# Alxaline/BraTS21

Measured on AMD Instinct MI355X. Metric: train patches/sec (4x128^3, width-48), higher is better.
Workload: dtype bf16; 1 GPU; equiunet width=48, batch=2/GPU of 4x128^3 synthetic patches, fwd + deep-supervision Dice + bwd + ranger (BASELINE.json configs[1]); global_batch=2, parallelism=dp1

## Files before the change

brats21_amd/csrc/gen_twin_dispatch.py:

```python
#!/usr/bin/env python3
import re
import sys

BOTH = {"brats_conv3d_set_vs8", "brats_conv3d_set_kp", "brats_conv3d_set_wgrad_alltaps", "brats_conv3d_set_x3_wgrad_fused"}
DATA = {"brats_conv3d_f8_fwd", "brats_conv3d_wgrad_f8", "brats_conv3d_pack_weights_multi"}

txt = re.sub(r"/\*.*?\*/", " ", open(sys.argv[1]).read(), flags=re.S)
protos = {}
for m in re.finditer(r"(const char\s*\*|size_t|int)\s+(brats_[a-z0-9_]+)\s*\(([^)]*)\)\s*;", txt):
    protos[m.group(2)] = (" ".join(m.group(1).split()), " ".join(m.group(3).split()))
names = []
for path in sys.argv[2:]:
    for m in re.finditer(r'extern "C" [a-z_ \*]+?BRATS_API\((brats_[a-z0-9_]+)\)\(', open(path).read()):
        names.append(m.group(1))
print("// GENERATED by gen_twin_dispatch.py from include/brats_hip.h -- do not edit")
print('#include "../../include/brats_hip.h"')
print('extern "C" {')
for n in names:
    if n not in protos:
        raise SystemExit(f"{n} is defined in a twinned translation unit but not declared in brats_hip.h")
    ret, args = protos[n]
    arglist = [] if args in ("", "void") else [a.strip() for a in args.split(",")]
    argnames = [re.search(r"([A-Za-z_][A-Za-z0-9_]*)$", a).group(1) for a in arglist]
    call = ", ".join(argnames)
    sig = args if arglist else "void"
    print(f"{ret} {n}_bf16({sig});")
    print(f"{ret} {n}_f16({sig});")
    if n in DATA:
        if n + "_f16" not in protos:
            raise SystemExit(f"{n}_f16 must be declared in brats_hip.h (16-bit data, no dtype argument)")
        print(f"{ret} {n}({sig}) {{ return {n}_bf16({call}); }}")
    elif n in BOTH:
        print(f"{ret} {n}({sig}) {{ {n}_f16({call}); return {n}_bf16({call}); }}")
    elif "dtype" in argnames:
        call16 = ", ".join("BRATS_BF16" if a == "dtype" else a for a in argnames)
        callx3 = ", ".join("BRATS_X3_BF16" if a == "dtype" else a for a in argnames)
        print(f"{ret} {n}({sig}) {{ return dtype == BRATS_F16 ? {n}_f16({call16}) : dtype == BRATS_X3_F16 ? {n}_f16({callx3}) : {n}_bf16({call}); }}")
# ... 4 lines not shown
```

brats21_amd/csrc/head.hip:

```cpp
#include "twin_begin.hpp"
#include "common.hpp"

int brats_lerp_adjoint_f32_planes(const float* in, float* out, size_t outer, int Lout, int Lin, size_t inner, hipStream_t st);

static inline int sgrid(size_t total, int block) {
  size_t b = (total + block - 1) / block;
  return (int)(b < 1 ? 1 : (b > 8192 ? 8192 : b));
}
constexpr int HEAD_KMAX = 4;

struct HeadPre { const float* scale_shift; float nslope; int evo; };
DEVI float head_pre(float x, float sc, float sh, const HeadPre& pre) {
  if (pre.evo) return x * __builtin_amdgcn_rcpf(1.f + __expf(-x)) * sc + sh;
  const float p = x * sc + sh;
  return p > 0.f ? p : p * pre.nslope;
}
template <typename T, bool PRE = false>
__global__ void head_conv_kernel(const T* __restrict__ x, int xpitch, const float* __restrict__ w, const float* __restrict__ b,
                                 float* __restrict__ low, int C, int K, size_t voxels, HeadPre pre) {
  constexpr int VW = 16 / sizeof(T);
  extern __shared__ float sm[];
  float* ws = sm;
  float* red = sm + HEAD_KMAX * C;
  for (int i = threadIdx.x; i < K * C; i += blockDim.x) ws[i] = w[i];
  __syncthreads();
  const int n = blockIdx.y;
  const int cv = C / VW, vl_n = blockDim.x / cv;
  const int mycv = threadIdx.x % cv, myvl = threadIdx.x / cv, c0 = mycv * VW;
  const T* xb = x + (size_t)n * voxels * xpitch;
  float psc[VW], psh[VW];
  if constexpr (PRE) {
#pragma unroll
    for (int j = 0; j < VW; ++j) {
      const bool in = myvl < vl_n;
      psc[j] = in ? pre.scale_shift[((size_t)n * C + c0 + j) * 2] : 0.f;
      psh[j] = in ? pre.scale_shift[((size_t)n * C + c0 + j) * 2 + 1] : 0.f;
// ... 101 lines not shown
      for (int i = 0; i < 4; ++i) { xb0[i] = pre_act(xb0[i], 0); xb1[i] = pre_act(xb1[i], 1); }
    }
#pragma unroll
    for (int i = 0; i < 4; ++i) {
      f32x4 acc = {0.f, 0.f, 0.f, 0.f};
#pragma unroll
      for (int part = 2; part >= 0; --part) {
        acc = MFMA16_16x16x32(wa[part][0], xb0[i], acc);
        acc = MFMA16_16x16x32(wa[part][1], xb1[i], acc);
      }
      const size_t vv = v0 + 16 * i + v;
      if (q == 0 && vv < voxels) {
#pragma unroll
        for (int r = 0; r < 4; ++r)
          if (r < K) lowp[(size_t)r * voxels + vv] = acc[r] + bias[r];
      }
    }
  }
}

struct Lerp { int i0, i1; float w0, w1; };
DEVI Lerp lerp_coef(int o, int in_len, float scale) {
  const float src = scale * (float)o;
  Lerp l;
  l.i0 = (int)src;
  if (l.i0 > in_len - 1) l.i0 = in_len - 1;
  l.i1 = l.i0 + (l.i0 < in_len - 1 ? 1 : 0);
  l.w1 = fminf(fmaxf(src - (float)l.i0, 0.f), 1.f);
  l.w0 = 1.f - l.w1;
  return l;
}
static inline float ac_scale(int in_len, int out_len) { return out_len > 1 ? (float)(in_len - 1) / (float)(out_len - 1) : 0.f; }

__global__ void __launch_bounds__(256) upsample_planes_kernel(const float* __restrict__ low, float* __restrict__ out, int D, int H, int W, int sc,
                                                              float sd, float sh, float sw) {
  const int Ho = H * sc, Wo = W * sc, Do = D * sc, W4 = Wo / 4;
  const int zo = blockIdx.y;
  const size_t pl = blockIdx.z;
  const Lerp lz = lerp_coef(zo, D, sd);
  const float* p0 = low + pl * D * H * W + (size_t)lz.i0 * H * W;
  const float* p1 = low + pl * D * H * W + (size_t)lz.i1 * H * W;
  float* o = out + (pl * Do + zo) * (size_t)Ho * Wo;
  for (int it = blockIdx.x * blockDim.x + threadIdx.x; it < Ho * W4; it += gridDim.x * blockDim.x) {
    const int yo = it / W4, x0 = (it % W4) * 4;
    const Lerp ly = lerp_coef(yo, H, sh);
    f32x4 r;
#pragma unroll
    for (int j = 0; j < 4; ++j) {
      const Lerp lx = lerp_coef(x0 + j, W, sw);
      float acc = 0.f;
#pragma unroll
      for (int k = 0; k < 8; ++k) {
        const float* p = (k & 4) ? p1 : p0;
        const int yy = (k & 2) ? ly.i1 : ly.i0, xx = (k & 1) ? lx.i1 : lx.i0;
        const float wgt = ((k & 4) ? lz.w1 : lz.w0) * ((k & 2) ? ly.w1 : ly.w0) * ((k & 1) ? lx.w1 : lx.w0);
        acc += wgt * p[yy * W + xx];
      }
      r[j] = acc;
    }
    *(f32x4*)(o + (size_t)yo * Wo + x0) = r;
  }
}

template <bool PRE>
static int head_conv_launch(const void* x, int xpitch, const float* w, const float* b, float* low, int dtype, int N, int C, int K,
                            size_t vox, HeadPre pre, hipStream_t st) {
  const int vw = dtype == BRATS_BF16 ? 8 : 4;
  const int cvh = C / vw, vlh = 256 / cvh;
  if (cvh > 256) BRATS_FAIL(BRATS_E_UNSUPPORTED, "head_fwd: C too large");
  dim3 grid(sgrid((vox + vlh - 1) / vlh, 1), N);
  const size_t ldsh = (size_t)(HEAD_KMAX * C + 256 * HEAD_KMAX) * sizeof(float);
  if (dtype == BRATS_BF16 && C <= 64 && (double)vox * xpitch * 2 < 2147483648.0) {
    const size_t waves = (vox + 63) / 64;
    const unsigned gx = (unsigned)(waves / 4 < 1 ? 1 : (waves / 4 > 8192 ? 8192 : waves / 4));
    hipLaunchKernelGGL(head_conv_mfma_kernel<PRE>, dim3(gx, N), dim3(256), 0, st, (const bf16_t*)x, xpitch, w, b, low, C, K, vox, pre);
  } else if (dtype == BRATS_BF16)
    hipLaunchKernelGGL((head_conv_kernel<bf16_t, PRE>), grid, dim3(256), ldsh, st, (const bf16_t*)x, xpitch, w, b, low, C, K, vox, pre);
  else
    hipLaunchKernelGGL((head_conv_kernel<float, PRE>), grid, dim3(256), ldsh, st, (const float*)x, xpitch, w, b, low, C, K, vox, pre);
  BRATS_CHECK_LAUNCH();
  return 0;
}

extern "C" int BRATS_API(brats_gn_head_fwd)(const void* y, int ypitch, const float* scale_shift, int act, float slope, const float* w,
                                 const float* b, float* out, int dtype, int N, int C, int K, int voxels, brats_stream_t s) {
  const int vw = dtype == BRATS_BF16 ? 8 : 4;
  if (!y || !scale_shift || !w || !out || K < 1 || K > HEAD_KMAX || C % vw || ypitch % vw)
    BRATS_FAIL(BRATS_E_ARG, "gn_head_fwd: bad argument (K<=4, C multiple of %d)", vw);
  if (act > BRATS_ACT_LEAKY) BRATS_FAIL(BRATS_E_UNSUPPORTED, "gn_head_fwd: relu / leakyrelu only (act=%d)", act);
  return head_conv_launch<true>(y, ypitch, w, b, out, dtype, N, C, K, (size_t)voxels,
                                HeadPre{scale_shift, act == BRATS_ACT_RELU ? 0.f : slope, 0}, (hipStream_t)s);
}

extern "C" int BRATS_API(brats_evonorm_head_fwd)(const void* y, int ypitch, const float* scale_shift, const float* w, const float* b,
                                      float* out, int dtype, int N, int C, int K, int voxels, brats_stream_t s) {
  const int vw = dtype == BRATS_BF16 ? 8 : 4;
  if (!y || !scale_shift || !w || !out || K < 1 || K > HEAD_KMAX || C % vw || ypitch % vw)
    BRATS_FAIL(BRATS_E_ARG, "evonorm_head_fwd: bad argument (K<=4, C multiple of %d)", vw);
  return head_conv_launch<true>(y, ypitch, w, b, out, dtype, N, C, K, (size_t)voxels, HeadPre{scale_shift, 0.f, 1}, (hipStream_t)s);
}

extern "C" int BRATS_API(brats_head_fwd)(const void* x, int xpitch, const float* w, const float* b, float* lowres, float* out,
                              int dtype, int N, int C, int K, int D, int H, int W, int scale, brats_stream_t s) {
  const int vw = dtype == BRATS_BF16 ? 8 : 4;
  if (!x || !w || !out || K < 1 || K > HEAD_KMAX || C % vw || xpitch % vw || scale < 1)
    BRATS_FAIL(BRATS_E_ARG, "head_fwd: bad argument (K<=4, C multiple of %d)", vw);
  if (scale > 1 && !lowres) BRATS_FAIL(BRATS_E_ARG, "head_fwd: lowres workspace required when scale > 1");
  hipStream_t st = (hipStream_t)s;
  const size_t vox = (size_t)D * H * W;
  float* low = scale > 1 ? lowres : out;
  if (int rc = head_conv_launch<false>(x, xpitch, w, b, low, dtype, N, C, K, vox, HeadPre{nullptr, 0.f, 0}, st)) return rc;
  if (scale > 1) {
    if ((W * scale) % 4) BRATS_FAIL(BRATS_E_UNSUPPORTED, "head_fwd: up-sampled width %d must be a multiple of 4", W * scale);
    const int items = H * scale * (W * scale / 4);
    hipLaunchKernelGGL(upsample_planes_kernel, dim3((unsigned)((items + 255) / 256), (unsigned)(D * scale), (unsigned)(N * K)), dim3(256), 0, st,
                       (const float*)low, out, D, H, W, scale, ac_scale(D, D * scale), ac_scale(H, H * scale), ac_scale(W, W * scale));
  }
  BRATS_CHECK_LAUNCH();
  return 0;
}

template <typename T>
__global__ void __launch_bounds__(256) head_bwd_kernel(const T* __restrict__ x, int xpitch, const float* __restrict__ w, const float* __restrict__ dlow,
                                T* __restrict__ dx, int dxpitch, float* __restrict__ dw , int C, int K,
                                size_t voxels) {
  constexpr int VW = 16 / sizeof(T);
  extern __shared__ float sm[];
  float* ws = sm;
  for (int i = threadIdx.x; i < K * C; i += blockDim.x) ws[i] = w[i];
  __syncthreads();
  const int n = blockIdx.y;
  const int cv = C / VW, vl_n = blockDim.x / cv;
  const int mycv = threadIdx.x % cv, myvl = threadIdx.x / cv, c0 = mycv * VW;
  float aw[HEAD_KMAX][VW];
  float ab[HEAD_KMAX];
#pragma unroll
  for (int k = 0; k < HEAD_KMAX; ++k) {
    ab[k] = 0.f;
#pragma unroll
    for (int j = 0; j < VW; ++j) aw[k][j] = 0.f;
  }
  if (myvl < vl_n) {
    const T* xb = x + (size_t)n * voxels * xpitch + c0;
    T* dxb = dx ? dx + (size_t)n * voxels * dxpitch + c0 : nullptr;
    float wr[HEAD_KMAX][VW];
#pragma unroll
    for (int k = 0; k < HEAD_KMAX; ++k)
#pragma unroll
      for (int j = 0; j < VW; ++j) wr[k][j] = k < K ? ws[k * C + c0 + j] : 0.f;
// ... 57 lines not shown
  if ((int)threadIdx.x < K) {
    float t = 0.f;
    for (int l = 0; l < vl_n; ++l) t += scr[vl_n * K * C + l * K + threadIdx.x];
    part[K * C + threadIdx.x] = t;
  }
}

constexpr int HEAD_MAX_BLOCKS = 1024;
static size_t head_lerp_floats(int N, int K, int D, int H, int W, int scale) {
  if (scale <= 1) return 0;
  const size_t p = (size_t)N * K;
  const size_t dlow = p * D * H * W, t1 = p * D * (H * scale) * (W * scale), t2 = p * D * H * (W * scale);
  return dlow + t1 + t2;
}
extern "C" size_t BRATS_API(brats_head_bwd_ws_bytes)(int N, int C, int K, int D, int H, int W, int scale) {
  return (head_lerp_floats(N, K, D, H, W, scale) + (size_t)(N * HEAD_MAX_BLOCKS + 1) * (K * C + K)) * sizeof(float);
}

extern "C" int BRATS_API(brats_head_bwd)(const void* x, int xpitch, const float* w, const float* dout, float* ws, void* dx, int dxpitch,
                              float* dw, float* db, int dtype, int N, int C, int K, int D, int H, int W, int scale,
                              brats_stream_t s) {
  const int vw = dtype == BRATS_BF16 ? 8 : 4;
  if (!x || !w || !dout || !dw || !db || K < 1 || K > HEAD_KMAX || C % vw || xpitch % vw || (dx && dxpitch % vw) ||
      C / vw > 128)
    BRATS_FAIL(BRATS_E_ARG, "head_bwd: bad argument");
  if (!ws) BRATS_FAIL(BRATS_E_ARG, "head_bwd: workspace required");
  hipStream_t st = (hipStream_t)s;
  const size_t vox = (size_t)D * H * W, p = (size_t)N * K;
  const float* dlow = dout;
  if (scale > 1) {
    float* dl = ws;
    float* t1 = dl + p * vox;
    float* t2 = t1 + p * D * (H * scale) * (W * scale);
    int rc;
    if ((rc = brats_lerp_adjoint_f32_planes(dout, t1, p, D * scale, D, (size_t)H * scale * W * scale, st))) return rc;
    if ((rc = brats_lerp_adjoint_f32_planes(t1, t2, p * D, H * scale, H, (size_t)W * scale, st))) return rc;
    if ((rc = brats_lerp_adjoint_f32_planes(t2, dl, p * D * H, W * scale, W, 1, st))) return rc;
    dlow = dl;
  }
  const int cv = C / vw, vl = 256 / cv;
  size_t gx = (vox + (size_t)vl * 16 - 1) / ((size_t)vl * 16);
  dim3 grid((unsigned)(gx < 1 ? 1 : (gx > HEAD_MAX_BLOCKS ? HEAD_MAX_BLOCKS : gx)), N);
  const size_t lds = (size_t)(K * C + vl * K * C + vl * K) * sizeof(float);
  float* part = ws + head_lerp_floats(N, K, D, H, W, scale);
  float* tot = part + (size_t)N * HEAD_MAX_BLOCKS * (K * C + K);
  if (dtype == BRATS_BF16)
    hipLaunchKernelGGL(head_bwd_kernel<bf16_t>, grid, dim3(256), lds, st, (const bf16_t*)x, xpitch, w, dlow, (bf16_t*)dx,
                       dxpitch, part, C, K, vox);
  else
    hipLaunchKernelGGL(head_bwd_kernel<float>, grid, dim3(256), lds, st, (const float*)x, xpitch, w, dlow, (float*)dx, dxpitch,
                       part, C, K, vox);
  (void)tot;
  brats_ordered_sum2(part, dw, K * C, db, N * (int)grid.x, K * C + K, st);
  BRATS_CHECK_LAUNCH();
  return 0;
}
#include "twin_end.hpp"
```

brats21_amd/csrc/pool_up.hip:

```cpp
#include "twin_begin.hpp"
#include "common.hpp"

static inline int stream_grid(size_t total, int block) {
  size_t b = (total + block - 1) / block;
  return (int)(b < 1 ? 1 : (b > 8192 ? 8192 : b));
}

template <typename T>
__global__ void maxpool2_fwd_kernel(const T* __restrict__ x, int xpitch, T* __restrict__ y, int ypitch, int N, int C,
                                    int D, int H, int W, int with_avg, uint8_t* __restrict__ argmax) {
  constexpr int VW = 16 / sizeof(T);
  const int cv = C / VW, Do = D / 2, Ho = H / 2, Wo = W / 2;
  const size_t total = (size_t)N * Do * Ho * Wo * cv;
  for (size_t it = (size_t)blockIdx.x * blockDim.x + threadIdx.x; it < total; it += (size_t)gridDim.x * blockDim.x) {
    const int c0 = (int)(it % cv) * VW;
    size_t v = it / cv;
    const int xo = v % Wo; v /= Wo;
    const int yo = v % Ho; v /= Ho;
    const int zo = v % Do;
    const int n = (int)(v / Do);
    float mx[VW], sm[VW];
    int am[VW];
#pragma unroll
    for (int j = 0; j < VW; ++j) { mx[j] = -INFINITY; sm[j] = 0.f; am[j] = 0; }
// ... 411 lines not shown
    for (int l = lo; l <= hi; ++l) {
      const Lerp c = lerp_coef(l, Lin, scale);
      float w = 0.f;
      if (c.i0 == i) w += c.w0;
      if (c.i1 == i) w += c.w1;
      if (w != 0.f) {
        float a[VW];
        if constexpr (VW == 1) a[0] = to_f<TI>(in[((o * Lout + l) * inner_vox + iv) * in_pitch + c0]);
        else Vec<TI, VW>::load(in + ((o * Lout + l) * inner_vox + iv) * in_pitch + c0, a);
#pragma unroll
        for (int j = 0; j < VW; ++j) acc[j] += w * a[j];
      }
    }
    if constexpr (VW == 1) out[((o * Lin + i) * inner_vox + iv) * out_pitch + c0] = from_f<TO>(acc[0]);
    else Vec<TO, VW>::store(out + ((o * Lin + i) * inner_vox + iv) * out_pitch + c0, acc);
  }
}

int brats_lerp_adjoint_f32_planes(const float* in, float* out, size_t outer, int Lout, int Lin, size_t inner,
                                  hipStream_t st) {
  const size_t total = outer * Lin * inner;
  if (inner % 4 == 0 && (((size_t)in | (size_t)out) & 15) == 0) {
    hipLaunchKernelGGL((lerp_adjoint_kernel<float, float, 4>), dim3(stream_grid(total / 4, 256)), dim3(256), 0, st, in, 4, out, 4,
                       outer, Lout, Lin, inner / 4, 4, ac_scale(Lin, Lout));
    BRATS_CHECK_LAUNCH();
    return 0;
  }
  hipLaunchKernelGGL((lerp_adjoint_kernel<float, float, 1>), dim3(stream_grid(total, 256)), dim3(256), 0, st, in, 1, out, 1,
                     outer, Lout, Lin, inner, 1, ac_scale(Lin, Lout));
  BRATS_CHECK_LAUNCH();
  return 0;
}

extern "C" size_t BRATS_API(brats_upsample_bwd_ws_bytes)(int dtype, int N, int C, int D, int H, int W, int scale) {
  const size_t esz = dtype == BRATS_BF16 ? 2 : 4;
  const size_t a = (size_t)N * D * (H * scale) * (W * scale) * C;
  const size_t b = (size_t)N * D * H * (W * scale) * C;
  return ((a * esz + 255) / 256 * 256) + ((b * esz + 255) / 256 * 256);
}

template <typename T>
static int upsample_bwd_t(const T* dy, int dypitch, T* dx, int dxpitch, char* tmp, int N, int C, int D, int H, int W, int sc,
                          hipStream_t st) {
  constexpr int VW = 16 / sizeof(T);
  const int Do = D * sc, Ho = H * sc, Wo = W * sc;
  const size_t a_elems = (size_t)N * D * Ho * Wo * C;
  T* t1 = (T*)tmp;
  T* t2 = (T*)(tmp + ((a_elems * sizeof(T) + 255) / 256 * 256));
  size_t total = (size_t)N * D * Ho * Wo * (C / VW);
  hipLaunchKernelGGL((lerp_adjoint_kernel<T, T, VW>), dim3(stream_grid(total, 256)), dim3(256), 0, st, dy, dypitch, t1, C,
                     (size_t)N, Do, D, (size_t)Ho * Wo, C, ac_scale(D, Do));
  total = (size_t)N * D * H * Wo * (C / VW);
  hipLaunchKernelGGL((lerp_adjoint_kernel<T, T, VW>), dim3(stream_grid(total, 256)), dim3(256), 0, st, (const T*)t1, C, t2, C,
                     (size_t)N * D, Ho, H, (size_t)Wo, C, ac_scale(H, Ho));
  total = (size_t)N * D * H * W * (C / VW);
  hipLaunchKernelGGL((lerp_adjoint_kernel<T, T, VW>), dim3(stream_grid(total, 256)), dim3(256), 0, st, (const T*)t2, C, dx,
                     dxpitch, (size_t)N * D * H, Wo, W, (size_t)1, C, ac_scale(W, Wo));
  BRATS_CHECK_LAUNCH();
  return 0;
}

extern "C" int BRATS_API(brats_upsample_bwd)(const void* dy, int dypitch, void* dx, int dxpitch, void* tmp, int dtype, int N, int C,
                                  int D, int H, int W, int scale, brats_stream_t s) {
  const int vw = dtype == BRATS_BF16 ? 8 : 4;
  if (!dy || !dx || !tmp || C % vw || dypitch % vw || dxpitch % vw) BRATS_FAIL(BRATS_E_ARG, "upsample_bwd: bad argument");
  if (dtype == BRATS_BF16)
    return upsample_bwd_t<bf16_t>((const bf16_t*)dy, dypitch, (bf16_t*)dx, dxpitch, (char*)tmp, N, C, D, H, W, scale,
                                  (hipStream_t)s);
  return upsample_bwd_t<float>((const float*)dy, dypitch, (float*)dx, dxpitch, (char*)tmp, N, C, D, H, W, scale,
                               (hipStream_t)s);
}
#include "twin_end.hpp"
```

brats21_amd/ops.py:

```python
import contextlib
import weakref

import numpy as np
import torch

from . import _lib
from ._lib import ACT_LEAKY, ACT_NONE, ACT_RELU, BF16, F16, F32, PACK_DGRAD, PACK_FWD, X3_BF16, X3_F16

ACTS = {"none": ACT_NONE, "relu": ACT_RELU, "leakyrelu": ACT_LEAKY, "elu": _lib.ACT_ELU, "swish": _lib.ACT_SWISH,
        "mish": _lib.ACT_MISH}


class KernelTimer:

    def __init__(self):
        self.records = {}

    def span(self, key):
        return _Span(self, key)

    def summary(self):
        torch.cuda.synchronize()
        out = {}
        for key, evs in self.records.items():
# ... 764 lines not shown
        x._pool_argmax = idx
    return out


def maxpool2_bwd(x, dy, dx_skip=None, with_avg=False):
    ptr, c, p = _desc(x)
    dptr, _, dp = _desc(dy)
    n, d, h, w, _ = x.shape
    dx = new_act(n, d, h, w, c, x.dtype, x.device)
    sptr, sp = (None, 0)
    if dx_skip is not None:
        sptr, _, sp = _desc(dx_skip)
    idx = getattr(x, "_pool_argmax", None)
    if idx is not None:
        _lib.check(_lib.lib().brats_maxpool2_bwd_idx(idx.data_ptr(), dptr, dp, sptr, sp, dx.data_ptr(), c, _code(x.dtype), n, c,
                                                     d, h, w, int(with_avg), _stream()), "maxpool2_bwd_idx")
        return dx
    _lib.check(_lib.lib().brats_maxpool2_bwd(ptr, p, None, 0, dptr, dp, sptr, sp, dx.data_ptr(), c, _code(x.dtype), n, c,
                                             d, h, w, int(with_avg), _stream()), "maxpool2_bwd")
    return dx


def upsample(x, scale=2, out=None):
    ptr, c, p = _desc(x)
    n, d, h, w, _ = x.shape
    if out is None:
        out = new_act(n, d * scale, h * scale, w * scale, c, x.dtype, x.device)
    optr, oc, op = _desc(out)
    _lib.check(_lib.lib().brats_upsample_fwd(ptr, p, optr, op, _code(x.dtype), n, c, d, h, w, scale, _stream()),
               "upsample_fwd")
    return out


def upsample_bwd(dy, scale=2):
    dptr, c, dp = _desc(dy)
    n, do, ho, wo, _ = dy.shape
    d, h, w = do // scale, ho // scale, wo // scale
    code = _code(dy.dtype)
    ws = torch.empty(_lib.lib().brats_upsample_bwd_ws_bytes(code, n, c, d, h, w, scale), dtype=torch.uint8, device=dy.device)
    dx = new_act(n, d, h, w, c, dy.dtype, dy.device)
    _lib.check(_lib.lib().brats_upsample_bwd(dptr, dp, dx.data_ptr(), c, ws.data_ptr(), code, n, c, d, h, w, scale,
                                             _stream()), "upsample_bwd")
    return dx


def head(x, weight, bias, scale=1):
    ptr, c, p = _desc(x)
    n, d, h, w, _ = x.shape
    k = weight.shape[0]
    wf = weight.detach().reshape(k, c).contiguous().float()
    out = torch.empty((n, k, d * scale, h * scale, w * scale), dtype=torch.float32, device=x.device)
    low = torch.empty((n, k, d, h, w), dtype=torch.float32, device=x.device) if scale > 1 else None
    _lib.check(_lib.lib().brats_head_fwd(ptr, p, wf.data_ptr(), _f32(bias.detach()) if bias is not None else None,
                                         low.data_ptr() if low is not None else None, out.data_ptr(), _code(x.dtype), n, c,
                                         k, d, h, w, scale, _stream()), "head_fwd")
    return out


def gn_head(y, scale_shift, weight, bias, act="relu", slope=0.01):
    ptr, c, p = _desc(y)
    n, d, h, w, _ = y.shape
    k = weight.shape[0]
    wf = weight.detach().reshape(k, c).contiguous().float()
    out = torch.empty((n, k, d, h, w), dtype=torch.float32, device=y.device)
    _lib.check(_lib.lib().brats_gn_head_fwd(ptr, p, scale_shift.data_ptr(), ACTS[act], slope, wf.data_ptr(),
                                            _f32(bias.detach()) if bias is not None else None, out.data_ptr(), _code(y.dtype), n, c,
# ... 321 lines not shown
```

include/brats_hip.h:

```cpp
#ifndef BRATS_HIP_H
#define BRATS_HIP_H
#include <stddef.h>
#include <stdint.h>

#ifdef __cplusplus
extern "C" {
#endif

typedef void* brats_stream_t;

enum { BRATS_F32 = 0, BRATS_BF16 = 1, BRATS_F16 = 2, BRATS_X3_BF16 = 3, BRATS_X3_F16 = 4 };
enum { BRATS_E_ARG = -1, BRATS_E_UNSUPPORTED = -2, BRATS_E_HIP = -3 };
enum { BRATS_ACT_NONE = 0, BRATS_ACT_RELU = 1, BRATS_ACT_LEAKY = 2, BRATS_ACT_ELU = 3, BRATS_ACT_SWISH = 4, BRATS_ACT_MISH = 5 };

#define BRATS_ABI_VERSION 7
int brats_abi_version(void);
const char* brats_last_error(void);

int brats_dropout(const void* x, int xpitch, void* out, int opitch, int dtype, size_t voxels, int C, float p,
                  const void* state, int unit, brats_stream_t s);

int brats_ncdhw_to_ndhwc(const float* src, void* dst, int dtype, int N, int C, int cpad, int dst_pitch,
                         int D, int H, int W, brats_stream_t s);
int brats_ndhwc_to_ncdhw(const void* src, int src_pitch, float* dst, int dtype, int N, int C,
// ... 155 lines not shown
                              float* amax, brats_stream_t s);
int brats_evonorm_se_fwd(const void* x, int xpitch, const float* mean_rstd, const float* gamma, const float* beta,
                         const float* w1, const float* b1, const float* w2, const float* b2, void* out, int opitch,
                         float* ws, float* chansum_out, float* gate1p, float* hidden, int Ch, int dtype, int N, int voxels,
                         int C, int groups, float* amax ,
                         brats_stream_t s);
int brats_channel_dot(const void* a, int apitch, const void* b , int bpitch, float* out ,
                      int dtype, int N, int voxels, int C, brats_stream_t s);
int brats_channel_scale(const void* a, int apitch, const float* scale , const float* add ,
                        void* dst, int dpitch, int dtype, int N, int voxels, int C,
                        float* amax , brats_stream_t s);
typedef struct { const void* x; const void* w; int xpitch, cin, ksize, dil; } brats_dconv_term;
typedef struct { brats_dconv_term term[4]; int nterms, rows; const float* bias; void* y; int ypitch, reserved; } brats_dconv_job;
size_t brats_dconv_packed_bytes(int dtype, int ksize, int kdim, int rows);
int brats_dconv_pack_weights(const float* w, void* packed, int dtype, int mode, int ksize, int cout_w, int cin_w,
                             int cin_off, int cin_cnt, brats_stream_t s);
int brats_dconv_run(const brats_dconv_job* jobs, int njobs, int dtype, int N, int D, int H, int W, brats_stream_t s);

int brats_maxpool2_fwd(const void* x, int xpitch, void* y, int ypitch,
                       unsigned char* argmax ,
                       int dtype, int N, int C, int D, int H, int W, int with_avg, brats_stream_t s);
int brats_maxpool2_bwd(const void* x, int xpitch, const void* y, int ypitch, const void* dy, int dypitch,
                       const void* dx_skip, int dxskip_pitch, void* dx, int dxpitch, int dtype,
                       int N, int C, int D, int H, int W, int with_avg, brats_stream_t s);
int brats_maxpool2_bwd_idx(const unsigned char* argmax, const void* dy, int dypitch, const void* dx_skip ,
                           int dxskip_pitch, void* dx, int dxpitch, int dtype, int N, int C, int D, int H, int W,
                           int with_avg, brats_stream_t s);

int brats_upsample_fwd(const void* x, int xpitch, void* y, int ypitch, int dtype, int N, int C,
                       int D, int H, int W, int scale, brats_stream_t s);
size_t brats_upsample_bwd_ws_bytes(int dtype, int N, int C, int D, int H, int W, int scale);
int brats_upsample_bwd(const void* dy, int dypitch, void* dx, int dxpitch, void* tmp, int dtype,
                       int N, int C, int D, int H, int W, int scale, brats_stream_t s);

int brats_head_fwd(const void* x, int xpitch, const float* w , const float* b, float* lowres ,
                   float* out , int dtype, int N, int C, int K,
                   int D, int H, int W, int scale, brats_stream_t s);
int brats_gn_head_fwd(const void* y, int ypitch, const float* scale_shift, int act, float slope, const float* w ,
                      const float* b, float* out, int dtype, int N, int C, int K, int voxels, brats_stream_t s);
int brats_evonorm_head_fwd(const void* y, int ypitch, const float* scale_shift, const float* w , const float* b,
                           float* out, int dtype, int N, int C, int K, int voxels, brats_stream_t s);
size_t brats_head_bwd_ws_bytes(int N, int C, int K, int D, int H, int W, int scale);
int brats_head_bwd(const void* x, int xpitch, const float* w, const float* dout, float* ws,
                   void* dx, int dxpitch, float* dw, float* db, int dtype, int N, int C, int K,
                   int D, int H, int W, int scale, brats_stream_t s);

int brats_sw_gather(const float* src, float* dst, const int* windows, int B, int C, int D, int H, int W,
                    int rd, int rh, int rw, int pad_z, int pad_y, int pad_x, float cval, int pad_mode, brats_stream_t s);
int brats_sw_accumulate(const float* prob, const float* importance, float* out, float* count, int K,
                        int Dp, int Hp, int Wp, int rd, int rh, int rw, int n, int z0, int y0, int x0,
                        brats_stream_t s);
int brats_sw_accumulate_multi(const float* prob, const float* importance, float* out, float* count, const int* windows,
                              int B, int NB, int K, int Dp, int Hp, int Wp, int rd, int rh, int rw, brats_stream_t s);
int brats_sw_finalize(const float* out, const float* count, float* dst, int NK, int Dp, int Hp, int Wp,
                      int D, int H, int W, int pad_z, int pad_y, int pad_x, brats_stream_t s);

int brats_spatial_signed_perm(const float* src, float* dst, int planes, int s0, int s1, int s2,
                              int p0, int p1, int p2, int f0, int f1, int f2, int mode, brats_stream_t s);

size_t brats_dice_ws_floats(int N, int K);
int brats_dice_stats(const float* logits, const float* target, float* sums , float* ws, int N, int K,
                     size_t voxels, brats_stream_t s);
int brats_dice_grad(const float* logits, const float* target, const float* coef ,
                    float* dlogits, int N, int K, size_t voxels, brats_stream_t s);

int brats_pad_crop(const float* src, float* dst, int planes, int sd, int sh, int sw, int dd, int dh,
// ... 72 lines not shown
```

Measured before the change: 133.5 patches/s.

## Fuse separable trilinear upsample backward passes and tile head upsample through LDS

Replaces the three separable lerp-adjoint passes in upsample backward (bf16 channels-last and f32 head planes) with single fused kernels. These stream depth planes with register accumulators and reduce H and W through LDS, which removes two full-size intermediate tensors and their global round trips. The head forward upsample now stages low-res rows and x-interpolation coefficients in shared memory instead of recomputing them and gathering from global memory. The cost is added kernel complexity, LDS use and occupancy limits, plus shape constraints; unsupported shapes fall back to the old path.

```diff
diff --git a/brats21_amd/csrc/gen_twin_dispatch.py b/brats21_amd/csrc/gen_twin_dispatch.py
--- a/brats21_amd/csrc/gen_twin_dispatch.py
+++ b/brats21_amd/csrc/gen_twin_dispatch.py
@@ -2,7 +2,8 @@
 import re
 import sys
 
-BOTH = {"brats_conv3d_set_vs8", "brats_conv3d_set_kp", "brats_conv3d_set_wgrad_alltaps", "brats_conv3d_set_x3_wgrad_fused"}
+BOTH = {"brats_conv3d_set_vs8", "brats_conv3d_set_kp", "brats_conv3d_set_wgrad_alltaps", "brats_conv3d_set_x3_wgrad_fused",
+        "brats_upsample_bwd_set_fused"}
 DATA = {"brats_conv3d_f8_fwd", "brats_conv3d_wgrad_f8", "brats_conv3d_pack_weights_multi"}
 
 txt = re.sub(r"/\*.*?\*/", " ", open(sys.argv[1]).read(), flags=re.S)
diff --git a/brats21_amd/csrc/head.hip b/brats21_amd/csrc/head.hip
--- a/brats21_amd/csrc/head.hip
+++ b/brats21_amd/csrc/head.hip
@@ -2,6 +2,7 @@
 #include "common.hpp"
 
 int brats_lerp_adjoint_f32_planes(const float* in, float* out, size_t outer, int Lout, int Lin, size_t inner, hipStream_t st);
+int brats_planes_adjoint_f32(const float* in, float* out, size_t P, int D, int H, int W, int sc, hipStream_t st);
 
 static inline int sgrid(size_t total, int block) {
   size_t b = (total + block - 1) / block;
@@ -169,29 +170,56 @@
 }
 static inline float ac_scale(int in_len, int out_len) { return out_len > 1 ? (float)(in_len - 1) / (float)(out_len - 1) : 0.f; }
 
+constexpr int UPL_ROWS = 32;
+static inline int upl_nlow(int sc) { return UPL_ROWS / sc + 3; }
 __global__ void __launch_bounds__(256) upsample_planes_kernel(const float* __restrict__ low, float* __restrict__ out, int D, int H, int W, int sc,
-                                                              float sd, float sh, float sw) {
-  const int Ho = H * sc, Wo = W * sc, Do = D * sc, W4 = Wo / 4;
-  const int zo = blockIdx.y;
+                                                              int nlow, float sd, float sh, float sw) {
+  extern __shared__ __attribute__((aligned(16))) float upl[];
+  const int Ho = H * sc, Wo = W * sc, Do = D * sc, W4 = Wo / 4, Wp = W + 1;
+  float* lows = upl;
+  int* xi = (int*)(upl + (2 * nlow * Wp + 3) / 4 * 4);
+  float* xw0 = (float*)(xi + Wo);
+  float* xw1 = xw0 + Wo;
+  const int zo = blockIdx.y, y0 = blockIdx.x * UPL_ROWS;
+  const int rows = Ho - y0 < UPL_ROWS ? Ho - y0 : UPL_ROWS;
   const size_t pl = blockIdx.z;
   const Lerp lz = lerp_coef(zo, D, sd);
-  const float* p0 = low + pl * D * H * W + (size_t)lz.i0 * H * W;
-  const float* p1 = low + pl * D * H * W + (size_t)lz.i1 * H * W;
+  const int ylo = lerp_coef(y0, H, sh).i0;
+  int cnt = lerp_coef(y0 + rows - 1, H, sh).i1 - ylo + 1;
+  if (cnt > nlow) cnt = nlow;
+  const float* p0 = low + pl * D * H * W + (size_t)lz.i0 * H * W + (size_t)ylo * W;
+  const float* p1 = low + pl * D * H * W + (size_t)lz.i1 * H * W + (size_t)ylo * W;
+  for (int idx = threadIdx.x; idx < 2 * cnt * Wp; idx += blockDim.x) {
+    const int pz = idx / (cnt * Wp), rem = idx % (cnt * Wp), r = rem / Wp, x = rem % Wp;
+    lows[(pz * nlow + r) * Wp + x] = (pz ? p1 : p0)[r * W + (x < W ? x : W - 1)];
+  }
+  for (int x = threadIdx.x; x < Wo; x += blockDim.x) {
+    const Lerp lx = lerp_coef(x, W, sw);
+    xi[x] = lx.i0;
+    xw0[x] = lx.w0;
+    xw1[x] = lx.w1;
+  }
+  __syncthreads();
   float* o = out + (pl * Do + zo) * (size_t)Ho * Wo;
-  for (int it = blockIdx.x * blockDim.x + threadIdx.x; it < Ho * W4; it += gridDim.x * blockDim.x) {
-    const int yo = it / W4, x0 = (it % W4) * 4;
+  typedef __attribute__((ext_vector_type(4))) int i32x4;
+  for (int it = threadIdx.x; it < rows * W4; it += blockDim.x) {
+    const int yo = y0 + it / W4, x0 = (it % W4) * 4;
     const Lerp ly = lerp_coef(yo, H, sh);
+    const float wzy[4] = {lz.w0 * ly.w0, lz.w0 * ly.w1, lz.w1 * ly.w0, lz.w1 * ly.w1};
+    int r0 = ly.i0 - ylo, r1 = ly.i1 - ylo;
+    r0 = r0 < cnt ? r0 : cnt - 1;
+    r1 = r1 < cnt ? r1 : cnt - 1;
+    const float* rp[4] = {lows + r0 * Wp, lows + r1 * Wp, lows + (nlow + r0) * Wp, lows + (nlow + r1) * Wp};
+    const i32x4 i0 = *(const i32x4*)(xi + x0);
+    const f32x4 w0 = *(const f32x4*)(xw0 + x0), w1 = *(const f32x4*)(xw1 + x0);
     f32x4 r;
 #pragma unroll
     for (int j = 0; j < 4; ++j) {
-      const Lerp lx = lerp_coef(x0 + j, W, sw);
       float acc = 0.f;
 #pragma unroll
       for (int k = 0; k < 8; ++k) {
-        const float* p = (k & 4) ? p1 : p0;
-        const int yy = (k & 2) ? ly.i1 : ly.i0, xx = (k & 1) ? lx.i1 : lx.i0;
-        const float wgt = ((k & 4) ? lz.w1 : lz.w0) * ((k & 2) ? ly.w1 : ly.w0) * ((k & 1) ? lx.w1 : lx.w0);
-        acc += wgt * p[yy * W + xx];
+        const float wgt = wzy[k >> 1] * ((k & 1) ? w1[j] : w0[j]);
+        acc += wgt * rp[k >> 1][i0[j] + (k & 1)];
       }
       r[j] = acc;
     }
@@ -249,9 +277,12 @@
   if (int rc = head_conv_launch<false>(x, xpitch, w, b, low, dtype, N, C, K, vox, HeadPre{nullptr, 0.f, 0}, st)) return rc;
   if (scale > 1) {
     if ((W * scale) % 4) BRATS_FAIL(BRATS_E_UNSUPPORTED, "head_fwd: up-sampled width %d must be a multiple of 4", W * scale);
-    const int items = H * scale * (W * scale / 4);
-    hipLaunchKernelGGL(upsample_planes_kernel, dim3((unsigned)((items + 255) / 256), (unsigned)(D * scale), (unsigned)(N * K)), dim3(256), 0, st,
-                       (const float*)low, out, D, H, W, scale, ac_scale(D, D * scale), ac_scale(H, H * scale), ac_scale(W, W * scale));
+    const int nlow = upl_nlow(scale);
+    const size_t lds = ((size_t)(2 * nlow * (W + 1) + 3) / 4 * 4 + (size_t)3 * W * scale) * sizeof(float);
+    if (lds > 64 * 1024 || D * scale > 65535 || N * K > 65535) BRATS_FAIL(BRATS_E_UNSUPPORTED, "head_fwd: planes of width %d x scale %d are too large", W, scale);
+    hipLaunchKernelGGL(upsample_planes_kernel, dim3((unsigned)((H * scale + UPL_ROWS - 1) / UPL_ROWS), (unsigned)(D * scale), (unsigned)(N * K)),
+                       dim3(256), lds, st, (const float*)low, out, D, H, W, scale, nlow, ac_scale(D, D * scale), ac_scale(H, H * scale),
+                       ac_scale(W, W * scale));
   }
   BRATS_CHECK_LAUNCH();
   return 0;
@@ -375,10 +406,13 @@
     float* dl = ws;
     float* t1 = dl + p * vox;
     float* t2 = t1 + p * D * (H * scale) * (W * scale);
-    int rc;
-    if ((rc = brats_lerp_adjoint_f32_planes(dout, t1, p, D * scale, D, (size_t)H * scale * W * scale, st))) return rc;
-    if ((rc = brats_lerp_adjoint_f32_planes(t1, t2, p * D, H * scale, H, (size_t)W * scale, st))) return rc;
-    if ((rc = brats_lerp_adjoint_f32_planes(t2, dl, p * D * H, W * scale, W, 1, st))) return rc;
+    int rc = brats_planes_adjoint_f32(dout, dl, p, D, H, W, scale, st);
+    if (rc < 0) return rc;
+    if (rc > 0) {
+      if ((rc = brats_lerp_adjoint_f32_planes(dout, t1, p, D * scale, D, (size_t)H * scale * W * scale, st))) return rc;
+      if ((rc = brats_lerp_adjoint_f32_planes(t1, t2, p * D, H * scale, H, (size_t)W * scale, st))) return rc;
+      if ((rc = brats_lerp_adjoint_f32_planes(t2, dl, p * D * H, W * scale, W, 1, st))) return rc;
+    }
     dlow = dl;
   }
   const int cv = C / vw, vl = 256 / cv;
diff --git a/brats21_amd/csrc/pool_up.hip b/brats21_amd/csrc/pool_up.hip
--- a/brats21_amd/csrc/pool_up.hip
+++ b/brats21_amd/csrc/pool_up.hip
@@ -467,6 +467,335 @@
   return 0;
 }
 
+
+DEVI void lerp_fine_range(int a, int cnt, int Lin, int Lout, float scale, int& lo, int& hi) {
+  const float inv = scale > 0.f ? 1.f / scale : 0.f;
+  lo = (int)floorf((float)(a - 1) * inv) - 2;
+  hi = (int)ceilf((float)(a + cnt) * inv) + 2;
+  if (scale <= 0.f) { lo = 0; hi = Lout - 1; }
+  lo = lo < 0 ? 0 : lo;
+  hi = hi > Lout - 1 ? Lout - 1 : hi;
+  while (lo < hi && lerp_coef(lo, Lin, scale).i1 < a) ++lo;
+  while (hi > lo && lerp_coef(hi, Lin, scale).i0 > a + cnt - 1) --hi;
+}
+DEVI float lerp_weight_to(int l, int i, int Lin, float scale) {
+  const Lerp c = lerp_coef(l, Lin, scale);
+  float w = 0.f;
+  if (c.i0 == i) w += c.w0;
+  if (c.i1 == i) w += c.w1;
+  return w;
+}
+
+constexpr int UBF_TH = 4, UBF_TW = 8, UBF_FH = 12, UBF_FW = 20, UBF_CS = 48, UBF_CV = UBF_CS / 8, UBF_THREADS = 512, UBF_KC = 3, UBF_MAXP = 2;
+static_assert(UBF_FH * UBF_FW * UBF_CV <= UBF_THREADS * UBF_KC, "every column of the fine footprint needs a thread slot");
+DEVI void ubf_add(float* acc, float w, const bf16_t* p) {
+  float a[8];
+  Vec<bf16_t, 8>::load(p, a);
+#pragma unroll
+  for (int j = 0; j < 8; ++j) acc[j] += w * a[j];
+}
+struct UbfStep { int l[UBF_MAXP]; float wc[UBF_MAXP], wn[UBF_MAXP]; int np; };
+__global__ void __launch_bounds__(UBF_THREADS, 4) upsample2_bwd_fused_kernel(const bf16_t* __restrict__ dy, int dypitch, bf16_t* __restrict__ dx,
+                                                                          int dxpitch, int C, int D, int H, int W, int cd, float sd,
+                                                                          float sh, float sw) {
+  __shared__ __attribute__((aligned(16))) bf16_t slab[UBF_FH * UBF_FW * UBF_CS];
+  __shared__ __attribute__((aligned(16))) bf16_t t2s[UBF_TH * UBF_FW * UBF_CS];
+  __shared__ float wys[UBF_TH][UBF_FH], wxs[UBF_TW][UBF_FW];
+  __shared__ int yrng[UBF_TH][2], xrng[UBF_TW][2];
+  const int Do = 2 * D, Ho = 2 * H, Wo = 2 * W;
+  const int nsl = C / UBF_CS, tiles_x = W / UBF_TW, tiles_y = H / UBF_TH, nz = D / cd;
+  int bid = blockIdx.x;
+  if (gridDim.x % 8 == 0) bid = (bid % 8) * (gridDim.x / 8) + bid / 8;
+  const int sl = bid % nsl, tx = (bid / nsl) % tiles_x, ty = (bid / (nsl * tiles_x)) % tiles_y;
+  const int zc = (bid / (nsl * tiles_x * tiles_y)) % nz, n = bid / (nsl * tiles_x * tiles_y * nz);
+  const int za = zc * cd, ya = ty * UBF_TH, xa = tx * UBF_TW;
+  const int tid = threadIdx.x;
+  int yl, yh, xl, xh;
+  lerp_fine_range(ya, UBF_TH, H, Ho, sh, yl, yh);
+  lerp_fine_range(xa, UBF_TW, W, Wo, sw, xl, xh);
+  if (yh - yl + 1 > UBF_FH) yh = yl + UBF_FH - 1;
+  if (xh - xl + 1 > UBF_FW) xh = xl + UBF_FW - 1;
+  const int fh = yh - yl + 1, fw = xh - xl + 1;
+  if (tid < UBF_TH * UBF_FH) {
+    const int t = tid / UBF_FH, f = tid % UBF_FH;
+    wys[t][f] = f < fh ? lerp_weight_to(yl + f, ya + t, H, sh) : 0.f;
+  } else if (tid >= 64 && tid < 64 + UBF_TW * UBF_FW) {
+    const int t = (tid - 64) / UBF_FW, f = (tid - 64) % UBF_FW;
+    wxs[t][f] = f < fw ? lerp_weight_to(xl + f, xa + t, W, sw) : 0.f;
+  }
+  __syncthreads();
+  if (tid < UBF_TH + UBF_TW) {
+    const int ax = tid >= UBF_TH, t = ax ? tid - UBF_TH : tid, fn = ax ? fw : fh;
+    const float* wt = ax ? wxs[t] : wys[t];
+    int a = 0, b = fn - 1;
+    while (a < b && wt[a] == 0.f) ++a;
+    while (b > a && wt[b] == 0.f) --b;
+    (ax ? xrng : yrng)[t][0] = a;
+    (ax ? xrng : yrng)[t][1] = b;
+  }
+  const int ncol = fh * fw * UBF_CV;
+  const bf16_t* src = dy + (size_t)n * Do * Ho * Wo * dypitch + (size_t)sl * UBF_CS;
+  const size_t plane = (size_t)Ho * Wo * dypitch;
+  size_t coloff[UBF_KC];
+  bool colok[UBF_KC];
+#pragma unroll
+  for (int k = 0; k < UBF_KC; ++k) {
+    const int col = tid + k * UBF_THREADS;
+    colok[k] = col < ncol;
+    const int cvi = col % UBF_CV, xx = (col / UBF_CV) % fw, yy = colok[k] ? col / (UBF_CV * fw) : 0;
+    coloff[k] = ((size_t)(yl + yy) * Wo + (xl + xx)) * dypitch + cvi * 8;
+  }
+  const int i_first = za > 0 ? za - 1 : 0, i_last = za + cd - 1;
+  int lcur, lend;
+  lerp_fine_range(i_first, 1, D, Do, sd, lcur, lend);
+  while (lcur < Do && lerp_coef(lcur, D, sd).i0 < i_first) ++lcur;
+  auto plan = [&](int i, UbfStep& st) {
+    st.np = 0;
+#pragma unroll
+    for (int p = 0; p < UBF_MAXP; ++p) {
+      st.l[p] = 0; st.wc[p] = 0.f; st.wn[p] = 0.f;
+      if (st.np == p && lcur < Do) {
+        const Lerp c = lerp_coef(lcur, D, sd);
+        if (c.i0 == i) {
+          st.l[p] = lcur;
+          st.wc[p] = c.i1 == i ? c.w0 + c.w1 : c.w0;
+          st.wn[p] = c.i1 == i + 1 ? c.w1 : 0.f;
+          st.np = p + 1;
+          ++lcur;
+        }
+      }
+    }
+  };
+  u32x4 raw[UBF_MAXP][UBF_KC];
+  auto issue = [&](const UbfStep& st) {
+#pragma unroll
+    for (int p = 0; p < UBF_MAXP; ++p)
+      if (p < st.np) {
+#pragma unroll
+        for (int k = 0; k < UBF_KC; ++k)
+          raw[p][k] = colok[k] ? *(const u32x4*)(src + (size_t)st.l[p] * plane + coloff[k]) : u32x4{0u, 0u, 0u, 0u};
+      }
+  };
+  float cur[UBF_KC][8], nxt[UBF_KC][8];
+#pragma unroll
+  for (int k = 0; k < UBF_KC; ++k)
+#pragma unroll
+    for (int j = 0; j < 8; ++j) { cur[k][j] = 0.f; nxt[k][j] = 0.f; }
+  auto accumulate = [&](const UbfStep& st) {
+#pragma unroll
+    for (int p = 0; p < UBF_MAXP; ++p)
+      if (p < st.np) {
+#pragma unroll
+        for (int k = 0; k < UBF_KC; ++k) {
+          float a[8];
+#pragma unroll
+          for (int q = 0; q < 4; ++q) unpack2(raw[p][k][q], a[2 * q], a[2 * q + 1]);
+          if (st.wc[p] != 0.f) {
+#pragma unroll
+            for (int j = 0; j < 8; ++j) cur[k][j] += st.wc[p] * a[j];
+          }
+          if (st.wn[p] != 0.f) {
+#pragma unroll
+            for (int j = 0; j < 8; ++j) nxt[k][j] += st.wn[p] * a[j];
+          }
+        }
+      }
+  };
+  UbfStep st;
+  plan(i_first, st);
+  issue(st);
+  bf16_t* dst = dx + (size_t)n * D * H * W * dxpitch + (size_t)sl * UBF_CS;
+  for (int i = i_first; i <= i_last; ++i) {
+    accumulate(st);
+    while (st.np == UBF_MAXP) {
+      plan(i, st);
+      issue(st);
+      accumulate(st);
+    }
+    if (i >= za) {
+#pragma unroll
+      for (int k = 0; k < UBF_KC; ++k)
+        if (colok[k]) Vec<bf16_t, 8>::store(slab + (size_t)(tid + k * UBF_THREADS) * 8, cur[k]);
+    }
+#pragma unroll
+    for (int k = 0; k < UBF_KC; ++k)
+#pragma unroll
+      for (int j = 0; j < 8; ++j) { cur[k][j] = nxt[k][j]; nxt[k][j] = 0.f; }
+    if (i < i_last) {
+      plan(i + 1, st);
+      issue(st);
+    } else {
+      st.np = 0;
+    }
+    __syncthreads();
+    if (i < za) continue;
+    const int rowv = fw * UBF_CV;
+    for (int it = tid; it < UBF_TH * rowv; it += UBF_THREADS) {
+      const int h = it / rowv, r = it % rowv;
+      float acc[8];
+#pragma unroll
+      for (int j = 0; j < 8; ++j) acc[j] = 0.f;
+      for (int f = yrng[h][0]; f <= yrng[h][1]; ++f) {
+        const float w = wys[h][f];
+        if (w != 0.f) ubf_add(acc, w, slab + ((size_t)f * rowv + r) * 8);
+      }
+      Vec<bf16_t, 8>::store(t2s + (size_t)it * 8, acc);
+    }
+    __syncthreads();
+    for (int it = tid; it < UBF_TH * UBF_TW * UBF_CV; it += UBF_THREADS) {
+      const int cvi = it % UBF_CV, xc = (it / UBF_CV) % UBF_TW, h = it / (UBF_CV * UBF_TW);
+      float acc[8];
+#pragma unroll
+      for (int j = 0; j < 8; ++j) acc[j] = 0.f;
+      for (int f = xrng[xc][0]; f <= xrng[xc][1]; ++f) {
+        const float w = wxs[xc][f];
+        if (w != 0.f) ubf_add(acc, w, t2s + ((size_t)(h * fw + f) * UBF_CV + cvi) * 8);
+      }
+      Vec<bf16_t, 8>::store(dst + (((size_t)i * H + ya + h) * W + xa + xc) * dxpitch + cvi * 8, acc);
+    }
+  }
+}
+
+static int g_upsample_bwd_fused = -1;
+extern "C" int BRATS_API(brats_upsample_bwd_set_fused)(int mode) {
+  const int old = g_upsample_bwd_fused;
+  g_upsample_bwd_fused = mode < 0 ? -1 : (mode ? 1 : 0);
+  return old;
+}
+static int upsample_bwd_fused_cd(int N, int C, int D, int H, int W, int sc) {
+  if (g_upsample_bwd_fused == 0 || sc != 2 || C % UBF_CS || H % UBF_TH || W % UBF_TW || D % 4) return 0;
+  const size_t per_z = (size_t)N * (H / UBF_TH) * (W / UBF_TW) * (C / UBF_CS);
+  int cd = 16;
+  while (cd > 4 && (D % cd || per_z * (D / cd) < 1024)) cd /= 2;
+  if (per_z * (D / cd) > 0x7fffffffull) return 0;
+  return cd;
+}
+
+constexpr int PAF_THREADS = 256;
+template <int KC, int B>
+__global__ void __launch_bounds__(PAF_THREADS) planes_adjoint_fused_kernel(const float* __restrict__ in, float* __restrict__ out, int D, int H, int W,
+                                                                           int sc, int cd, int th, int fmax, float sd, float sh, float sw) {
+  extern __shared__ __attribute__((aligned(16))) float paf_lds[];
+  const int Do = D * sc, Ho = H * sc, Wo = W * sc, W4 = Wo / 4;
+  float* t1s = paf_lds;
+  float* t2s = paf_lds + (size_t)cd * fmax * Wo;
+  const int ya = blockIdx.x * th, za = blockIdx.y * cd;
+  const size_t pl = blockIdx.z;
+  const int tid = threadIdx.x;
+  int yl, yh;
+  lerp_fine_range(ya, th, H, Ho, sh, yl, yh);
+  if (yh - yl + 1 > fmax) yh = yl + fmax - 1;
+  const int fh = yh - yl + 1;
+  const int ncol = fh * W4;
+  const float* src = in + pl * Do * Ho * Wo + (size_t)yl * Wo;
+  const size_t plane = (size_t)Ho * Wo;
+  const int i_first = za > 0 ? za - 1 : 0, i_last = za + cd - 1;
+  int lstart, lend;
+  lerp_fine_range(i_first, i_last - i_first + 1, D, Do, sd, lstart, lend);
+  while (lstart < lend && lerp_coef(lstart, D, sd).i0 < i_first) ++lstart;
+  f32x4 cur[KC], nxt[KC];
+#pragma unroll
+  for (int k = 0; k < KC; ++k) { cur[k] = f32x4{0.f, 0.f, 0.f, 0.f}; nxt[k] = cur[k]; }
+  int i = i_first;
+  auto flush = [&]() {
+#pragma unroll
+    for (int k = 0; k < KC; ++k) {
+      const int col = tid + k * PAF_THREADS;
+      if (i >= za && col < ncol) *(f32x4*)(t1s + ((size_t)(i - za) * fmax * W4 + col) * 4) = cur[k];
+      cur[k] = nxt[k];
+      nxt[k] = f32x4{0.f, 0.f, 0.f, 0.f};
+    }
+    ++i;
+  };
+  for (int l0 = lstart; l0 <= lend; l0 += B) {
+    f32x4 raw[B][KC];
+#pragma unroll
+    for (int b = 0; b < B; ++b)
+      if (l0 + b <= lend) {
+#pragma unroll
+        for (int k = 0; k < KC; ++k) {
+          const int col = tid + k * PAF_THREADS;
+          raw[b][k] = col < ncol ? *(const f32x4*)(src + (size_t)(l0 + b) * plane + (size_t)col * 4) : f32x4{0.f, 0.f, 0.f, 0.f};
+        }
+      }
+#pragma unroll
+    for (int b = 0; b < B; ++b)
+      if (l0 + b <= lend) {
+        const Lerp c = lerp_coef(l0 + b, D, sd);
+        while (i < c.i0 && i <= i_last) flush();
+        const float wc = c.i1 == i ? c.w0 + c.w1 : c.w0, wn = c.i1 == i + 1 ? c.w1 : 0.f;
+#pragma unroll
+        for (int k = 0; k < KC; ++k) {
+          if (wc != 0.f) {
+#pragma unroll
+            for (int j = 0; j < 4; ++j) cur[k][j] += wc * raw[b][k][j];
+          }
+          if (wn != 0.f) {
+#pragma unroll
+            for (int j = 0; j < 4; ++j) nxt[k][j] += wn * raw[b][k][j];
+          }
+        }
+      }
+  }
+  while (i <= i_last) flush();
+  __syncthreads();
+  const float invh = sh > 0.f ? 1.f / sh : 0.f, invw = sw > 0.f ? 1.f / sw : 0.f;
+  for (int it = tid; it < cd * th * W4; it += PAF_THREADS) {
+    const int x4 = it % W4, h = (it / W4) % th, z = it / (W4 * th), ic = ya + h;
+    int lo = (int)floorf((float)(ic - 1) * invh) - 1, hi = (int)ceilf((float)(ic + 1) * invh) + 1;
+    if (sh <= 0.f) { lo = 0; hi = Ho - 1; }
+    lo = lo < yl ? yl : lo;
+    hi = hi > yh ? yh : hi;
+    f32x4 acc = {0.f, 0.f, 0.f, 0.f};
+    for (int l = lo; l <= hi; ++l) {
+      const float w = lerp_weight_to(l, ic, H, sh);
+      if (w != 0.f) {
+        const f32x4 a = *(const f32x4*)(t1s + ((size_t)(z * fmax + l - yl) * W4 + x4) * 4);
+#pragma unroll
+        for (int j = 0; j < 4; ++j) acc[j] += w * a[j];
+      }
+    }
+    *(f32x4*)(t2s + (size_t)it * 4) = acc;
+  }
+  __syncthreads();
+  for (int it = tid; it < cd * th * W; it += PAF_THREADS) {
+    const int xc = it % W, h = (it / W) % th, z = it / (W * th);
+    int lo = (int)floorf((float)(xc - 1) * invw) - 1, hi = (int)ceilf((float)(xc + 1) * invw) + 1;
+    if (sw <= 0.f) { lo = 0; hi = Wo - 1; }
+    lo = lo < 0 ? 0 : lo;
+    hi = hi > Wo - 1 ? Wo - 1 : hi;
+    float acc = 0.f;
+    for (int l = lo; l <= hi; ++l) {
+      const float w = lerp_weight_to(l, xc, W, sw);
+      if (w != 0.f) acc += w * t2s[(size_t)(z * th + h) * Wo + l];
+    }
+    out[((pl * D + za + z) * H + ya + h) * (size_t)W + xc] = acc;
+  }
+}
+
+int brats_planes_adjoint_f32(const float* in, float* out, size_t P, int D, int H, int W, int sc, hipStream_t st) {
+  const int Wo = W * sc;
+  if (Wo % 4 || (((size_t)in | (size_t)out) & 15) || P > 65535 || D > 65535) return 1;
+  int cd = 16 / sc < 2 ? 2 : (16 / sc > 4 ? 4 : 16 / sc), th = 8 / sc < 2 ? 2 : (8 / sc > 4 ? 4 : 8 / sc);
+  while (cd > 1 && D % cd) cd /= 2;
+  while (th > 1 && H % th) th /= 2;
+  const float scale_h = H > 1 ? (float)(H - 1) / (float)(H * sc - 1) : 0.f;
+  int fmax = scale_h > 0.f ? (int)ceilf((float)(th + 1) / scale_h) + 2 : H * sc;
+  if (fmax > H * sc) fmax = H * sc;
+  const size_t lds = (size_t)cd * (fmax + th) * Wo * sizeof(float);
+  const int kc = (fmax * (Wo / 4) + PAF_THREADS - 1) / PAF_THREADS;
+  if (lds > 64 * 1024 || kc > 6) return 1;
+  const dim3 grid(H / th, D / cd, (unsigned)P);
+#define PAF_LAUNCH(KC, B) hipLaunchKernelGGL((planes_adjoint_fused_kernel<KC, B>), grid, dim3(PAF_THREADS), lds, st, in, out, D, H, W, sc, cd, th, \
+                                             fmax, ac_scale(D, D * sc), ac_scale(H, H * sc), ac_scale(W, W * sc))
+  if (kc <= 2) PAF_LAUNCH(2, 8);
+  else if (kc <= 4) PAF_LAUNCH(4, 4);
+  else PAF_LAUNCH(6, 2);
+#undef PAF_LAUNCH
+  BRATS_CHECK_LAUNCH();
+  return 0;
+}
+
 extern "C" size_t BRATS_API(brats_upsample_bwd_ws_bytes)(int dtype, int N, int C, int D, int H, int W, int scale) {
   const size_t esz = dtype == BRATS_BF16 ? 2 : 4;
   const size_t a = (size_t)N * D * (H * scale) * (W * scale) * C;
@@ -479,6 +808,15 @@
                           hipStream_t st) {
   constexpr int VW = 16 / sizeof(T);
   const int Do = D * sc, Ho = H * sc, Wo = W * sc;
+  if constexpr (sizeof(T) == 2) {
+    if (const int cd = upsample_bwd_fused_cd(N, C, D, H, W, sc)) {
+      const dim3 grid((unsigned)((size_t)N * (H / UBF_TH) * (W / UBF_TW) * (C / UBF_CS) * (D / cd)));
+      hipLaunchKernelGGL(upsample2_bwd_fused_kernel, grid, dim3(UBF_THREADS), 0, st, dy, dypitch, dx, dxpitch, C, D, H, W, cd,
+                         ac_scale(D, Do), ac_scale(H, Ho), ac_scale(W, Wo));
+      BRATS_CHECK_LAUNCH();
+      return 0;
+    }
+  }
   const size_t a_elems = (size_t)N * D * Ho * Wo * C;
   T* t1 = (T*)tmp;
   T* t2 = (T*)(tmp + ((a_elems * sizeof(T) + 255) / 256 * 256));
diff --git a/brats21_amd/ops.py b/brats21_amd/ops.py
--- a/brats21_amd/ops.py
+++ b/brats21_amd/ops.py
@@ -820,6 +820,10 @@
     return out
 
 
+def set_upsample_bwd_fused(mode):
+    return _lib.lib().brats_upsample_bwd_set_fused(mode)
+
+
 def upsample_bwd(dy, scale=2):
     dptr, c, dp = _desc(dy)
     n, do, ho, wo, _ = dy.shape
diff --git a/include/brats_hip.h b/include/brats_hip.h
--- a/include/brats_hip.h
+++ b/include/brats_hip.h
@@ -211,6 +211,7 @@
 size_t brats_upsample_bwd_ws_bytes(int dtype, int N, int C, int D, int H, int W, int scale);
 int brats_upsample_bwd(const void* dy, int dypitch, void* dx, int dxpitch, void* tmp, int dtype,
                        int N, int C, int D, int H, int W, int scale, brats_stream_t s);
+int brats_upsample_bwd_set_fused(int mode);
 
 int brats_head_fwd(const void* x, int xpitch, const float* w , const float* b, float* lowres ,
                    float* out , int dtype, int N, int C, int K,
```

New measurement: 135.8 patches/s (median of 6 runs). 1.7% higher.
